# alexandreGellibert/SDR-for-Android-lib

Measured on AMD Instinct MI355X. Metric: IQ Msamples/s (16384-pt FFT+SSB) at 1/2/4/8 GPUs; % HBM roofline, higher is better.
Workload: dtype f32 (int8 CS8 in, int16 PCM out)

## Files before the change

sdr-for-android-lib_amd/csrc/ssb.hip:

```cpp
#include <hip/hip_ext.h>
#include <stdio.h>
#include <stdlib.h>

#include <vector>

#include "pulse_front.h"
#include "sdrg_internal.h"
#include "ssb_common.h"
#include "ssb_lpf_asm.h"
#include "ssb_math.h"

#pragma clang fp contract(off)

namespace sdrg {
namespace {

constexpr int WAVE = 64;

struct Chain {
    float dc;
    float a0, a1, a2, b1, b2, z1, z2;
    float target, fast, gain;
    int upper;

// ... 355 lines not shown
                st_work += __builtin_amdgcn_s_memtime() - st_a;
            }
            lds_barrier();
        }
    };
    auto run = [&](int off, auto &&body) {
        chunk_loop([&](int it) {
            const int c = it - off;
            if (c >= 0 && c < nch) body(c);
        });
    };
    if ((skip_mask >> wave) & 1) {
        chunk_loop([&](int) {});
    } else if (wave == W_DC) {
        float dc = 0.0f;
        run(1, [&](int c) {
            const float alpha = 0.9995f, one_minus = 1.0f - 0.9995f, a0 = p.lpf[0];
            if (SDRG_DC_ASM && c >= 0 && c < nch && lane < PG) {
                const f2v om2 = {one_minus, one_minus}, a02 = {a0, a0};
                const uint32_t src = lds_addr(&L.re[c & 1][my_s * ROW]), dst = lds_addr(&L.a[c % NA][my_s * ROW]);
                if (SDRG_DC_ASM == 2)
                    asm volatile(SDRG_DC_CHUNK_IL_ASM
                                 : [dc] "+v"(dc)
                                 : [src] "v"(src), [dst] "v"(dst), [alpha] "s"(alpha), [om2] "s"(om2), [a02] "s"(a02)
                                 : SDRG_CHUNK_CLOBBERS, "memory");
                else
                    asm volatile(SDRG_DC_CHUNK_ASM
                                 : [dc] "+v"(dc)
                                 : [src] "v"(src), [dst] "v"(dst), [alpha] "s"(alpha), [om2] "s"(om2), [a02] "s"(a02)
                                 : SDRG_CHUNK_CLOBBERS, "memory");
            } else if (c >= 0 && c < nch && lane < PG) {
                row_pipeline(&L.re[c & 1][my_s * ROW], &L.a[c % NA][my_s * ROW], lane < PG, [&](float (&v)[SB]) {
#pragma unroll
                    for (int q = 0; q < SB; q++) {
                        dc = alpha * dc + one_minus * v[q];
                        v[q] = a0 * (v[q] - dc);
                    }
                });
            }
        });
    } else if (wave == W_LPF) {
        float z1 = 0.0f, z2 = 0.0f;
        const bool lpf_asm_loop = LA && SDRG_LPF_ASM && S % CH == 0;
        if (s0 + my_s < n_frames) {
            z1 = state[s0 + my_s].lpf_z1;
            z2 = state[s0 + my_s].lpf_z2;
        }
        const f2v c1 = {p.lpf[1], -p.lpf[3]}, c2 = {p.lpf[2], -p.lpf[4]};
        static_assert(BUFF * 4 == SDRG_LPF_LOOP_SLOT_BYTES, "ring slot stride of the generated loop");
        if (lpf_asm_loop) {
            f2v z = {z1, z2};
            const uint32_t abase = lds_addr(&L.a[0][my_s * ROW]), ybase = lds_addr(&L.y[0][my_s * ROW]);
            const int nit = nch + 8 + LA;
            unsigned long long sv;
            int t_it, t_cc, t_r, t_yo;
            if (SDRG_LPF_INTERLEAVE)
                asm volatile(SDRG_LPF_LOOP_IL_ASM
                             : [z] "+v"(z), [sv] "=&s"(sv), [it] "=&s"(t_it), [cc] "=&s"(t_cc), [r] "=&s"(t_r), [yo] "=&s"(t_yo)
                             : [abase] "v"(abase), [ybase] "v"(ybase), [c1] "s"(c1), [c2] "s"(c2), [nit] "s"(nit), [nch] "s"(nch)
                             : SDRG_CHUNK_CLOBBERS, "v54", "memory");
            else
                asm volatile(SDRG_LPF_LOOP_ASM
                             : [z] "+v"(z), [sv] "=&s"(sv), [it] "=&s"(t_it), [cc] "=&s"(t_cc), [r] "=&s"(t_r), [yo] "=&s"(t_yo)
                             : [abase] "v"(abase), [ybase] "v"(ybase), [c1] "s"(c1), [c2] "s"(c2), [nit] "s"(nit), [nch] "s"(nch)
                             : SDRG_CHUNK_CLOBBERS, "v54", "memory");
            z1 = z.x;
            z2 = z.y;
        } else run(2 + LA, [&](int c) {
            if (c >= 0 && c < nch && lane < PG) {
                const int lim = min(CH, S - c * CH);
                if (lim == CH && SDRG_LPF_ASM) {
                    f2v z = {z1, z2};
                    const uint32_t src = lds_addr(&L.a[c % NA][my_s * ROW]), dst = lds_addr(y_row(c, my_s));
                    asm volatile(SDRG_LPF_CHUNK_ASM
                                 : [z] "+v"(z)
                                 : [src] "v"(src), [dst] "v"(dst), [c1] "s"(c1), [c2] "s"(c2)
                                 : SDRG_LPF_CHUNK_CLOBBERS, "memory");
                    z1 = z.x;
                    z2 = z.y;
                } else if (lim == CH) {
                    row_pipeline(&L.a[c % NA][my_s * ROW], y_row(c, my_s), lane < PG, [&](float (&v)[SB]) {
#pragma unroll
                        for (int q = 0; q < SB; q++) {
                            const f2v p1 = c1 * z1, p2 = c2 * z2;
                            const float y = (((v[q] + p1.x) + p2.x) + p1.y) + p2.y;
                            z2 = z1;
                            z1 = y;
                            v[q] = y;
                        }
                    });
                } else {
                    for (int q = 0; q < lim; q++) {
                        const f2v p1 = c1 * z1, p2 = c2 * z2;
                        const float y = (((L.a[c % NA][my_s * ROW + q] + p1.x) + p2.x) + p1.y) + p2.y;
                        z2 = z1;
                        z1 = y;
                        if (lane < PG) y_row(c, my_s)[q] = y;
                    }
                }
            }
        });
        if (lane < PG && s0 + my_s < n_frames) {
            state[s0 + my_s].lpf_z1 = z1;
            state[s0 + my_s].lpf_z2 = z2;
        }
    } else if (wave == W_AGC) {
        float gain = 1.0f;
        const f2v rates = {p.agc_fast, 0.00035f};
        const f2v keep = {1.0f - p.agc_fast, 1.0f - 0.00035f};
        run(4 + LA, [&](int c) {
            if (SDRG_AGC_ASM && c >= 0 && c < nch && lane < PG) {
// ... 472 lines not shown
```

sdr-for-android-lib_amd/csrc/ssb_lpf_asm.h:

```cpp
#pragma once
#define SDRG_LPF_CHUNK_ASM \
    "ds_read_b128 v[0:3], %[src] offset:0\n" \
    "ds_read_b128 v[4:7], %[src] offset:16\n" \
    "ds_read_b128 v[8:11], %[src] offset:32\n" \
    "ds_read_b128 v[12:15], %[src] offset:48\n" \
    "ds_read_b128 v[16:19], %[src] offset:64\n" \
    "ds_read_b128 v[20:23], %[src] offset:80\n" \
    "ds_read_b128 v[24:27], %[src] offset:96\n" \
    "ds_read_b128 v[28:31], %[src] offset:112\n" \
    "s_waitcnt lgkmcnt(4)\n" \
    "v_pk_mul_f32 v[48:49], %[c1], %[z] op_sel:[0,0] op_sel_hi:[1,0]\n" \
    "v_pk_mul_f32 v[50:51], %[c2], %[z] op_sel:[0,1] op_sel_hi:[1,1]\n" \
    "v_add_f32 v0, v0, v48\n" \
    "v_add_f32 v0, v0, v50\n" \
    "v_add_f32 v0, v0, v49\n" \
    "v_add_f32 v0, v0, v51\n" \
    "v_pk_mul_f32 v[48:49], %[c1], v[0:1] op_sel:[0,0] op_sel_hi:[1,0]\n" \
    "v_pk_mul_f32 v[50:51], %[c2], %[z] op_sel:[0,0] op_sel_hi:[1,0]\n" \
    "v_add_f32 v1, v1, v48\n" \
    "v_add_f32 v1, v1, v50\n" \
    "v_add_f32 v1, v1, v49\n" \
    "v_add_f32 v1, v1, v51\n" \
    "v_pk_mul_f32 v[48:49], %[c1], v[0:1] op_sel:[0,1] op_sel_hi:[1,1]\n" \
    "v_pk_mul_f32 v[50:51], %[c2], v[0:1] op_sel:[0,0] op_sel_hi:[1,0]\n" \
// ... 2934 lines not shown
    "v_pk_mov_b32 v[52:53], v[46:47], v[46:47] op_sel:[1,0]\n" \
    "s_add_u32 %[yo], %[cc], 1\n" \
    "s_cmp_ge_i32 %[yo], %[nch]\n" \
    "s_cbranch_scc1 L_drain_%=\n" \
    "ds_read_b128 v[0:3], %[abase] offset:0\n" \
    "ds_read_b128 v[4:7], %[abase] offset:16\n" \
    "ds_read_b128 v[8:11], %[abase] offset:32\n" \
    "ds_read_b128 v[12:15], %[abase] offset:48\n" \
    "ds_read_b128 v[16:19], %[abase] offset:64\n" \
    "ds_read_b128 v[20:23], %[abase] offset:80\n" \
    "ds_read_b128 v[24:27], %[abase] offset:96\n" \
    "ds_read_b128 v[28:31], %[abase] offset:112\n" \
    "s_branch L_bar8_%=\n" \
    "L_pre_%=:\n" \
    "s_cmp_lg_i32 %[cc], -1\n" \
    "s_cbranch_scc1 L_drain_%=\n" \
    "s_cmp_le_i32 %[nch], 0\n" \
    "s_cbranch_scc1 L_drain_%=\n" \
    "ds_read_b128 v[0:3], %[abase] offset:0\n" \
    "ds_read_b128 v[4:7], %[abase] offset:16\n" \
    "ds_read_b128 v[8:11], %[abase] offset:32\n" \
    "ds_read_b128 v[12:15], %[abase] offset:48\n" \
    "ds_read_b128 v[16:19], %[abase] offset:64\n" \
    "ds_read_b128 v[20:23], %[abase] offset:80\n" \
    "ds_read_b128 v[24:27], %[abase] offset:96\n" \
    "ds_read_b128 v[28:31], %[abase] offset:112\n" \
    "L_bar8_%=:\n" \
    "s_waitcnt lgkmcnt(8)\n" \
    "s_branch L_bar_%=\n" \
    "L_drain_%=:\n" \
    "s_waitcnt lgkmcnt(0)\n" \
    "L_bar_%=:\n" \
    "s_barrier\n" \
    "s_add_u32 %[it], %[it], 1\n" \
    "s_add_i32 %[cc], %[cc], 1\n" \
    "s_cmp_le_i32 %[cc], 0\n" \
    "s_cbranch_scc1 L_next_%=\n" \
    "s_add_u32 %[r], %[r], 1\n" \
    "s_cmp_eq_u32 %[r], 3\n" \
    "s_cselect_b32 %[r], 0, %[r]\n" \
    "L_next_%=:\n" \
    "s_cmp_lt_u32 %[it], %[nit]\n" \
    "s_cbranch_scc1 L_top_%=\n" \
    "s_mov_b64 exec, %[sv]\n" \
    "s_nop 4\n" \
    "v_pk_mov_b32 %[z], v[52:53], v[52:53] op_sel:[0,1]\n" \
    ""
#define SDRG_LPF_LOOP_IL_ASM \
    "s_mov_b64 %[sv], exec\n" \
    "s_mov_b64 exec, 0xffff\n" \
    "s_nop 4\n" \
    "v_pk_mov_b32 v[46:47], %[z], %[z] op_sel:[1,0]\n" \
    "v_pk_mov_b32 v[52:53], %[z], %[z] op_sel:[0,1]\n" \
    "s_mov_b32 %[it], 0\n" \
    "s_mov_b32 %[cc], -3\n" \
    "s_mov_b32 %[r], 0\n" \
    "L_top_%=:\n" \
    "s_cmp_lt_i32 %[cc], 0\n" \
    "s_cbranch_scc1 L_pre_%=\n" \
    "s_cmp_ge_i32 %[cc], %[nch]\n" \
    "s_cbranch_scc1 L_drain_%=\n" \
    "s_and_b32 %[yo], %[cc], 3\n" \
    "s_mul_i32 %[yo], %[yo], 4352\n" \
    "v_add_u32 v54, %[yo], %[ybase]\n" \
    "s_cmp_eq_u32 %[r], 0\n" \
    "s_cbranch_scc1 L_r0_%=\n" \
    "s_cmp_eq_u32 %[r], 1\n" \
    "s_cbranch_scc1 L_r1_%=\n" \
    "s_branch L_r2_%=\n" \
    "L_r0_%=:\n" \
    "s_waitcnt lgkmcnt(4)\n" \
    "v_pk_mul_f32 v[48:49], %[c1], v[46:47] op_sel:[0,1] op_sel_hi:[1,1]\n" \
    "v_pk_mul_f32 v[50:51], %[c2], v[46:47] op_sel:[0,0] op_sel_hi:[1,0]\n" \
    "v_add_f32 v0, v0, v48\n" \
    "v_add_f32 v0, v0, v50\n" \
    "v_add_f32 v0, v0, v49\n" \
    "v_add_f32 v0, v0, v51\n" \
    "v_pk_mul_f32 v[48:49], %[c1], v[0:1] op_sel:[0,0] op_sel_hi:[1,0]\n" \
    "v_pk_mul_f32 v[50:51], %[c2], v[46:47] op_sel:[0,1] op_sel_hi:[1,1]\n" \
    "v_add_f32 v1, v1, v48\n" \
    "v_add_f32 v1, v1, v50\n" \
    "v_add_f32 v1, v1, v49\n" \
    "v_add_f32 v1, v1, v51\n" \
    "v_pk_mul_f32 v[48:49], %[c1], v[0:1] op_sel:[0,1] op_sel_hi:[1,1]\n" \
    "v_pk_mul_f32 v[50:51], %[c2], v[0:1] op_sel:[0,0] op_sel_hi:[1,0]\n" \
    "v_add_f32 v2, v2, v48\n" \
    "v_add_f32 v2, v2, v50\n" \
    "v_add_f32 v2, v2, v49\n" \
    "v_add_f32 v2, v2, v51\n" \
    "v_pk_mul_f32 v[48:49], %[c1], v[2:3] op_sel:[0,0] op_sel_hi:[1,0]\n" \
    "v_pk_mul_f32 v[50:51], %[c2], v[0:1] op_sel:[0,1] op_sel_hi:[1,1]\n" \
    "v_add_f32 v3, v3, v48\n" \
    "v_add_f32 v3, v3, v50\n" \
    "v_add_f32 v3, v3, v49\n" \
    "v_add_f32 v3, v3, v51\n" \
    "ds_write_b128 v54, v[0:3] offset:0\n" \
    "ds_read_b128 v[32:35], %[abase] offset:128\n" \
    "v_pk_mul_f32 v[48:49], %[c1], v[2:3] op_sel:[0,1] op_sel_hi:[1,1]\n" \
    "v_pk_mul_f32 v[50:51], %[c2], v[2:3] op_sel:[0,0] op_sel_hi:[1,0]\n" \
    "v_add_f32 v4, v4, v48\n" \
    "v_add_f32 v4, v4, v50\n" \
    "v_add_f32 v4, v4, v49\n" \
    "v_add_f32 v4, v4, v51\n" \
    "v_pk_mul_f32 v[48:49], %[c1], v[4:5] op_sel:[0,0] op_sel_hi:[1,0]\n" \
    "v_pk_mul_f32 v[50:51], %[c2], v[2:3] op_sel:[0,1] op_sel_hi:[1,1]\n" \
    "v_add_f32 v5, v5, v48\n" \
    "v_add_f32 v5, v5, v50\n" \
    "v_add_f32 v5, v5, v49\n" \
    "v_add_f32 v5, v5, v51\n" \
    "v_pk_mul_f32 v[48:49], %[c1], v[4:5] op_sel:[0,1] op_sel_hi:[1,1]\n" \
    "v_pk_mul_f32 v[50:51], %[c2], v[4:5] op_sel:[0,0] op_sel_hi:[1,0]\n" \
    "v_add_f32 v6, v6, v48\n" \
    "v_add_f32 v6, v6, v50\n" \
    "v_add_f32 v6, v6, v49\n" \
    "v_add_f32 v6, v6, v51\n" \
    "v_pk_mul_f32 v[48:49], %[c1], v[6:7] op_sel:[0,0] op_sel_hi:[1,0]\n" \
    "v_pk_mul_f32 v[50:51], %[c2], v[4:5] op_sel:[0,1] op_sel_hi:[1,1]\n" \
    "v_add_f32 v7, v7, v48\n" \
    "v_add_f32 v7, v7, v50\n" \
    "v_add_f32 v7, v7, v49\n" \
    "v_add_f32 v7, v7, v51\n" \
    "ds_write_b128 v54, v[4:7] offset:16\n" \
    "ds_read_b128 v[36:39], %[abase] offset:144\n" \
    "v_pk_mul_f32 v[48:49], %[c1], v[6:7] op_sel:[0,1] op_sel_hi:[1,1]\n" \
    "v_pk_mul_f32 v[50:51], %[c2], v[6:7] op_sel:[0,0] op_sel_hi:[1,0]\n" \
    "v_add_f32 v8, v8, v48\n" \
    "v_add_f32 v8, v8, v50\n" \
    "v_add_f32 v8, v8, v49\n" \
    "v_add_f32 v8, v8, v51\n" \
    "v_pk_mul_f32 v[48:49], %[c1], v[8:9] op_sel:[0,0] op_sel_hi:[1,0]\n" \
    "v_pk_mul_f32 v[50:51], %[c2], v[6:7] op_sel:[0,1] op_sel_hi:[1,1]\n" \
    "v_add_f32 v9, v9, v48\n" \
    "v_add_f32 v9, v9, v50\n" \
    "v_add_f32 v9, v9, v49\n" \
    "v_add_f32 v9, v9, v51\n" \
    "v_pk_mul_f32 v[48:49], %[c1], v[8:9] op_sel:[0,1] op_sel_hi:[1,1]\n" \
    "v_pk_mul_f32 v[50:51], %[c2], v[8:9] op_sel:[0,0] op_sel_hi:[1,0]\n" \
    "v_add_f32 v10, v10, v48\n" \
    "v_add_f32 v10, v10, v50\n" \
    "v_add_f32 v10, v10, v49\n" \
    "v_add_f32 v10, v10, v51\n" \
    "v_pk_mul_f32 v[48:49], %[c1], v[10:11] op_sel:[0,0] op_sel_hi:[1,0]\n" \
    "v_pk_mul_f32 v[50:51], %[c2], v[8:9] op_sel:[0,1] op_sel_hi:[1,1]\n" \
    "v_add_f32 v11, v11, v48\n" \
    "v_add_f32 v11, v11, v50\n" \
    "v_add_f32 v11, v11, v49\n" \
    "v_add_f32 v11, v11, v51\n" \
    "ds_write_b128 v54, v[8:11] offset:32\n" \
// ... 290 lines not shown
    "v_pk_mul_f32 v[48:49], %[c1], v[6:7] op_sel:[0,1] op_sel_hi:[1,1]\n" \
    "v_pk_mul_f32 v[50:51], %[c2], v[6:7] op_sel:[0,0] op_sel_hi:[1,0]\n" \
    "v_add_f32 v8, v8, v48\n" \
    "v_add_f32 v8, v8, v50\n" \
    "v_add_f32 v8, v8, v49\n" \
    "v_add_f32 v8, v8, v51\n" \
    "v_pk_mul_f32 v[48:49], %[c1], v[8:9] op_sel:[0,0] op_sel_hi:[1,0]\n" \
    "v_pk_mul_f32 v[50:51], %[c2], v[6:7] op_sel:[0,1] op_sel_hi:[1,1]\n" \
    "v_add_f32 v9, v9, v48\n" \
    "v_add_f32 v9, v9, v50\n" \
    "v_add_f32 v9, v9, v49\n" \
    "v_add_f32 v9, v9, v51\n" \
    "v_pk_mul_f32 v[48:49], %[c1], v[8:9] op_sel:[0,1] op_sel_hi:[1,1]\n" \
    "v_pk_mul_f32 v[50:51], %[c2], v[8:9] op_sel:[0,0] op_sel_hi:[1,0]\n" \
    "v_add_f32 v10, v10, v48\n" \
    "v_add_f32 v10, v10, v50\n" \
    "v_add_f32 v10, v10, v49\n" \
    "v_add_f32 v10, v10, v51\n" \
    "v_pk_mul_f32 v[48:49], %[c1], v[10:11] op_sel:[0,0] op_sel_hi:[1,0]\n" \
    "v_pk_mul_f32 v[50:51], %[c2], v[8:9] op_sel:[0,1] op_sel_hi:[1,1]\n" \
    "v_add_f32 v11, v11, v48\n" \
    "v_add_f32 v11, v11, v50\n" \
    "v_add_f32 v11, v11, v49\n" \
    "v_add_f32 v11, v11, v51\n" \
    "ds_write_b128 v54, v[8:11] offset:224\n" \
    "ds_read_b128 v[40:43], %[abase] offset:4448\n" \
    "v_pk_mul_f32 v[48:49], %[c1], v[10:11] op_sel:[0,1] op_sel_hi:[1,1]\n" \
    "v_pk_mul_f32 v[50:51], %[c2], v[10:11] op_sel:[0,0] op_sel_hi:[1,0]\n" \
    "v_add_f32 v12, v12, v48\n" \
    "v_add_f32 v12, v12, v50\n" \
    "v_add_f32 v12, v12, v49\n" \
    "v_add_f32 v12, v12, v51\n" \
    "v_pk_mul_f32 v[48:49], %[c1], v[12:13] op_sel:[0,0] op_sel_hi:[1,0]\n" \
    "v_pk_mul_f32 v[50:51], %[c2], v[10:11] op_sel:[0,1] op_sel_hi:[1,1]\n" \
    "v_add_f32 v13, v13, v48\n" \
    "v_add_f32 v13, v13, v50\n" \
    "v_add_f32 v13, v13, v49\n" \
    "v_add_f32 v13, v13, v51\n" \
    "v_pk_mul_f32 v[48:49], %[c1], v[12:13] op_sel:[0,1] op_sel_hi:[1,1]\n" \
    "v_pk_mul_f32 v[50:51], %[c2], v[12:13] op_sel:[0,0] op_sel_hi:[1,0]\n" \
    "v_add_f32 v14, v14, v48\n" \
    "v_add_f32 v14, v14, v50\n" \
    "v_add_f32 v14, v14, v49\n" \
    "v_add_f32 v14, v14, v51\n" \
    "v_pk_mul_f32 v[48:49], %[c1], v[14:15] op_sel:[0,0] op_sel_hi:[1,0]\n" \
    "v_pk_mul_f32 v[50:51], %[c2], v[12:13] op_sel:[0,1] op_sel_hi:[1,1]\n" \
    "v_add_f32 v15, v15, v48\n" \
    "v_add_f32 v15, v15, v50\n" \
    "v_add_f32 v15, v15, v49\n" \
    "v_add_f32 v15, v15, v51\n" \
    "ds_write_b128 v54, v[12:15] offset:240\n" \
    "ds_read_b128 v[44:47], %[abase] offset:4464\n" \
    "v_pk_mov_b32 v[52:53], v[14:15], v[14:15] op_sel:[1,0]\n" \
    "s_branch L_bar1_%=\n" \
    "L_r1_%=:\n" \
    "s_waitcnt lgkmcnt(4)\n" \
    "v_pk_mul_f32 v[48:49], %[c1], v[14:15] op_sel:[0,1] op_sel_hi:[1,1]\n" \
    "v_pk_mul_f32 v[50:51], %[c2], v[14:15] op_sel:[0,0] op_sel_hi:[1,0]\n" \
    "v_add_f32 v16, v16, v48\n" \
    "v_add_f32 v16, v16, v50\n" \
    "v_add_f32 v16, v16, v49\n" \
    "v_add_f32 v16, v16, v51\n" \
    "v_pk_mul_f32 v[48:49], %[c1], v[16:17] op_sel:[0,0] op_sel_hi:[1,0]\n" \
    "v_pk_mul_f32 v[50:51], %[c2], v[14:15] op_sel:[0,1] op_sel_hi:[1,1]\n" \
    "v_add_f32 v17, v17, v48\n" \
    "v_add_f32 v17, v17, v50\n" \
    "v_add_f32 v17, v17, v49\n" \
    "v_add_f32 v17, v17, v51\n" \
    "v_pk_mul_f32 v[48:49], %[c1], v[16:17] op_sel:[0,1] op_sel_hi:[1,1]\n" \
    "v_pk_mul_f32 v[50:51], %[c2], v[16:17] op_sel:[0,0] op_sel_hi:[1,0]\n" \
    "v_add_f32 v18, v18, v48\n" \
    "v_add_f32 v18, v18, v50\n" \
    "v_add_f32 v18, v18, v49\n" \
    "v_add_f32 v18, v18, v51\n" \
    "v_pk_mul_f32 v[48:49], %[c1], v[18:19] op_sel:[0,0] op_sel_hi:[1,0]\n" \
    "v_pk_mul_f32 v[50:51], %[c2], v[16:17] op_sel:[0,1] op_sel_hi:[1,1]\n" \
    "v_add_f32 v19, v19, v48\n" \
    "v_add_f32 v19, v19, v50\n" \
    "v_add_f32 v19, v19, v49\n" \
    "v_add_f32 v19, v19, v51\n" \
    "ds_write_b128 v54, v[16:19] offset:0\n" \
    "ds_read_b128 v[0:3], %[abase] offset:4480\n" \
    "v_pk_mul_f32 v[48:49], %[c1], v[18:19] op_sel:[0,1] op_sel_hi:[1,1]\n" \
    "v_pk_mul_f32 v[50:51], %[c2], v[18:19] op_sel:[0,0] op_sel_hi:[1,0]\n" \
    "v_add_f32 v20, v20, v48\n" \
    "v_add_f32 v20, v20, v50\n" \
    "v_add_f32 v20, v20, v49\n" \
    "v_add_f32 v20, v20, v51\n" \
    "v_pk_mul_f32 v[48:49], %[c1], v[20:21] op_sel:[0,0] op_sel_hi:[1,0]\n" \
    "v_pk_mul_f32 v[50:51], %[c2], v[18:19] op_sel:[0,1] op_sel_hi:[1,1]\n" \
    "v_add_f32 v21, v21, v48\n" \
    "v_add_f32 v21, v21, v50\n" \
    "v_add_f32 v21, v21, v49\n" \
    "v_add_f32 v21, v21, v51\n" \
    "v_pk_mul_f32 v[48:49], %[c1], v[20:21] op_sel:[0,1] op_sel_hi:[1,1]\n" \
    "v_pk_mul_f32 v[50:51], %[c2], v[20:21] op_sel:[0,0] op_sel_hi:[1,0]\n" \
    "v_add_f32 v22, v22, v48\n" \
    "v_add_f32 v22, v22, v50\n" \
    "v_add_f32 v22, v22, v49\n" \
    "v_add_f32 v22, v22, v51\n" \
    "v_pk_mul_f32 v[48:49], %[c1], v[22:23] op_sel:[0,0] op_sel_hi:[1,0]\n" \
    "v_pk_mul_f32 v[50:51], %[c2], v[20:21] op_sel:[0,1] op_sel_hi:[1,1]\n" \
    "v_add_f32 v23, v23, v48\n" \
    "v_add_f32 v23, v23, v50\n" \
    "v_add_f32 v23, v23, v49\n" \
    "v_add_f32 v23, v23, v51\n" \
    "ds_write_b128 v54, v[20:23] offset:16\n" \
    "ds_read_b128 v[4:7], %[abase] offset:4496\n" \
    "v_pk_mul_f32 v[48:49], %[c1], v[22:23] op_sel:[0,1] op_sel_hi:[1,1]\n" \
    "v_pk_mul_f32 v[50:51], %[c2], v[22:23] op_sel:[0,0] op_sel_hi:[1,0]\n" \
    "v_add_f32 v24, v24, v48\n" \
    "v_add_f32 v24, v24, v50\n" \
    "v_add_f32 v24, v24, v49\n" \
    "v_add_f32 v24, v24, v51\n" \
    "v_pk_mul_f32 v[48:49], %[c1], v[24:25] op_sel:[0,0] op_sel_hi:[1,0]\n" \
    "v_pk_mul_f32 v[50:51], %[c2], v[22:23] op_sel:[0,1] op_sel_hi:[1,1]\n" \
    "v_add_f32 v25, v25, v48\n" \
    "v_add_f32 v25, v25, v50\n" \
    "v_add_f32 v25, v25, v49\n" \
    "v_add_f32 v25, v25, v51\n" \
    "v_pk_mul_f32 v[48:49], %[c1], v[24:25] op_sel:[0,1] op_sel_hi:[1,1]\n" \
    "v_pk_mul_f32 v[50:51], %[c2], v[24:25] op_sel:[0,0] op_sel_hi:[1,0]\n" \
    "v_add_f32 v26, v26, v48\n" \
    "v_add_f32 v26, v26, v50\n" \
    "v_add_f32 v26, v26, v49\n" \
    "v_add_f32 v26, v26, v51\n" \
    "v_pk_mul_f32 v[48:49], %[c1], v[26:27] op_sel:[0,0] op_sel_hi:[1,0]\n" \
    "v_pk_mul_f32 v[50:51], %[c2], v[24:25] op_sel:[0,1] op_sel_hi:[1,1]\n" \
    "v_add_f32 v27, v27, v48\n" \
    "v_add_f32 v27, v27, v50\n" \
    "v_add_f32 v27, v27, v49\n" \
    "v_add_f32 v27, v27, v51\n" \
    "ds_write_b128 v54, v[24:27] offset:32\n" \
// ... 290 lines not shown
    "v_pk_mul_f32 v[48:49], %[c1], v[22:23] op_sel:[0,1] op_sel_hi:[1,1]\n" \
    "v_pk_mul_f32 v[50:51], %[c2], v[22:23] op_sel:[0,0] op_sel_hi:[1,0]\n" \
    "v_add_f32 v24, v24, v48\n" \
    "v_add_f32 v24, v24, v50\n" \
    "v_add_f32 v24, v24, v49\n" \
    "v_add_f32 v24, v24, v51\n" \
    "v_pk_mul_f32 v[48:49], %[c1], v[24:25] op_sel:[0,0] op_sel_hi:[1,0]\n" \
    "v_pk_mul_f32 v[50:51], %[c2], v[22:23] op_sel:[0,1] op_sel_hi:[1,1]\n" \
    "v_add_f32 v25, v25, v48\n" \
    "v_add_f32 v25, v25, v50\n" \
    "v_add_f32 v25, v25, v49\n" \
    "v_add_f32 v25, v25, v51\n" \
    "v_pk_mul_f32 v[48:49], %[c1], v[24:25] op_sel:[0,1] op_sel_hi:[1,1]\n" \
    "v_pk_mul_f32 v[50:51], %[c2], v[24:25] op_sel:[0,0] op_sel_hi:[1,0]\n" \
    "v_add_f32 v26, v26, v48\n" \
    "v_add_f32 v26, v26, v50\n" \
    "v_add_f32 v26, v26, v49\n" \
    "v_add_f32 v26, v26, v51\n" \
    "v_pk_mul_f32 v[48:49], %[c1], v[26:27] op_sel:[0,0] op_sel_hi:[1,0]\n" \
    "v_pk_mul_f32 v[50:51], %[c2], v[24:25] op_sel:[0,1] op_sel_hi:[1,1]\n" \
    "v_add_f32 v27, v27, v48\n" \
    "v_add_f32 v27, v27, v50\n" \
    "v_add_f32 v27, v27, v49\n" \
    "v_add_f32 v27, v27, v51\n" \
    "ds_write_b128 v54, v[24:27] offset:224\n" \
    "ds_read_b128 v[8:11], %[abase] offset:8800\n" \
    "v_pk_mul_f32 v[48:49], %[c1], v[26:27] op_sel:[0,1] op_sel_hi:[1,1]\n" \
    "v_pk_mul_f32 v[50:51], %[c2], v[26:27] op_sel:[0,0] op_sel_hi:[1,0]\n" \
    "v_add_f32 v28, v28, v48\n" \
    "v_add_f32 v28, v28, v50\n" \
    "v_add_f32 v28, v28, v49\n" \
    "v_add_f32 v28, v28, v51\n" \
    "v_pk_mul_f32 v[48:49], %[c1], v[28:29] op_sel:[0,0] op_sel_hi:[1,0]\n" \
    "v_pk_mul_f32 v[50:51], %[c2], v[26:27] op_sel:[0,1] op_sel_hi:[1,1]\n" \
    "v_add_f32 v29, v29, v48\n" \
    "v_add_f32 v29, v29, v50\n" \
    "v_add_f32 v29, v29, v49\n" \
    "v_add_f32 v29, v29, v51\n" \
    "v_pk_mul_f32 v[48:49], %[c1], v[28:29] op_sel:[0,1] op_sel_hi:[1,1]\n" \
    "v_pk_mul_f32 v[50:51], %[c2], v[28:29] op_sel:[0,0] op_sel_hi:[1,0]\n" \
    "v_add_f32 v30, v30, v48\n" \
    "v_add_f32 v30, v30, v50\n" \
    "v_add_f32 v30, v30, v49\n" \
    "v_add_f32 v30, v30, v51\n" \
    "v_pk_mul_f32 v[48:49], %[c1], v[30:31] op_sel:[0,0] op_sel_hi:[1,0]\n" \
    "v_pk_mul_f32 v[50:51], %[c2], v[28:29] op_sel:[0,1] op_sel_hi:[1,1]\n" \
    "v_add_f32 v31, v31, v48\n" \
    "v_add_f32 v31, v31, v50\n" \
    "v_add_f32 v31, v31, v49\n" \
    "v_add_f32 v31, v31, v51\n" \
    "ds_write_b128 v54, v[28:31] offset:240\n" \
    "ds_read_b128 v[12:15], %[abase] offset:8816\n" \
    "v_pk_mov_b32 v[52:53], v[30:31], v[30:31] op_sel:[1,0]\n" \
    "s_branch L_bar1_%=\n" \
    "L_r2_%=:\n" \
    "s_waitcnt lgkmcnt(4)\n" \
    "v_pk_mul_f32 v[48:49], %[c1], v[30:31] op_sel:[0,1] op_sel_hi:[1,1]\n" \
    "v_pk_mul_f32 v[50:51], %[c2], v[30:31] op_sel:[0,0] op_sel_hi:[1,0]\n" \
    "v_add_f32 v32, v32, v48\n" \
    "v_add_f32 v32, v32, v50\n" \
    "v_add_f32 v32, v32, v49\n" \
    "v_add_f32 v32, v32, v51\n" \
    "v_pk_mul_f32 v[48:49], %[c1], v[32:33] op_sel:[0,0] op_sel_hi:[1,0]\n" \
    "v_pk_mul_f32 v[50:51], %[c2], v[30:31] op_sel:[0,1] op_sel_hi:[1,1]\n" \
    "v_add_f32 v33, v33, v48\n" \
    "v_add_f32 v33, v33, v50\n" \
    "v_add_f32 v33, v33, v49\n" \
    "v_add_f32 v33, v33, v51\n" \
    "v_pk_mul_f32 v[48:49], %[c1], v[32:33] op_sel:[0,1] op_sel_hi:[1,1]\n" \
    "v_pk_mul_f32 v[50:51], %[c2], v[32:33] op_sel:[0,0] op_sel_hi:[1,0]\n" \
    "v_add_f32 v34, v34, v48\n" \
    "v_add_f32 v34, v34, v50\n" \
    "v_add_f32 v34, v34, v49\n" \
    "v_add_f32 v34, v34, v51\n" \
    "v_pk_mul_f32 v[48:49], %[c1], v[34:35] op_sel:[0,0] op_sel_hi:[1,0]\n" \
    "v_pk_mul_f32 v[50:51], %[c2], v[32:33] op_sel:[0,1] op_sel_hi:[1,1]\n" \
    "v_add_f32 v35, v35, v48\n" \
    "v_add_f32 v35, v35, v50\n" \
    "v_add_f32 v35, v35, v49\n" \
    "v_add_f32 v35, v35, v51\n" \
    "ds_write_b128 v54, v[32:35] offset:0\n" \
    "ds_read_b128 v[16:19], %[abase] offset:8832\n" \
    "v_pk_mul_f32 v[48:49], %[c1], v[34:35] op_sel:[0,1] op_sel_hi:[1,1]\n" \
    "v_pk_mul_f32 v[50:51], %[c2], v[34:35] op_sel:[0,0] op_sel_hi:[1,0]\n" \
    "v_add_f32 v36, v36, v48\n" \
    "v_add_f32 v36, v36, v50\n" \
    "v_add_f32 v36, v36, v49\n" \
    "v_add_f32 v36, v36, v51\n" \
    "v_pk_mul_f32 v[48:49], %[c1], v[36:37] op_sel:[0,0] op_sel_hi:[1,0]\n" \
    "v_pk_mul_f32 v[50:51], %[c2], v[34:35] op_sel:[0,1] op_sel_hi:[1,1]\n" \
    "v_add_f32 v37, v37, v48\n" \
    "v_add_f32 v37, v37, v50\n" \
    "v_add_f32 v37, v37, v49\n" \
    "v_add_f32 v37, v37, v51\n" \
    "v_pk_mul_f32 v[48:49], %[c1], v[36:37] op_sel:[0,1] op_sel_hi:[1,1]\n" \
    "v_pk_mul_f32 v[50:51], %[c2], v[36:37] op_sel:[0,0] op_sel_hi:[1,0]\n" \
    "v_add_f32 v38, v38, v48\n" \
    "v_add_f32 v38, v38, v50\n" \
    "v_add_f32 v38, v38, v49\n" \
    "v_add_f32 v38, v38, v51\n" \
    "v_pk_mul_f32 v[48:49], %[c1], v[38:39] op_sel:[0,0] op_sel_hi:[1,0]\n" \
    "v_pk_mul_f32 v[50:51], %[c2], v[36:37] op_sel:[0,1] op_sel_hi:[1,1]\n" \
    "v_add_f32 v39, v39, v48\n" \
    "v_add_f32 v39, v39, v50\n" \
    "v_add_f32 v39, v39, v49\n" \
    "v_add_f32 v39, v39, v51\n" \
    "ds_write_b128 v54, v[36:39] offset:16\n" \
    "ds_read_b128 v[20:23], %[abase] offset:8848\n" \
    "v_pk_mul_f32 v[48:49], %[c1], v[38:39] op_sel:[0,1] op_sel_hi:[1,1]\n" \
    "v_pk_mul_f32 v[50:51], %[c2], v[38:39] op_sel:[0,0] op_sel_hi:[1,0]\n" \
    "v_add_f32 v40, v40, v48\n" \
    "v_add_f32 v40, v40, v50\n" \
    "v_add_f32 v40, v40, v49\n" \
    "v_add_f32 v40, v40, v51\n" \
    "v_pk_mul_f32 v[48:49], %[c1], v[40:41] op_sel:[0,0] op_sel_hi:[1,0]\n" \
    "v_pk_mul_f32 v[50:51], %[c2], v[38:39] op_sel:[0,1] op_sel_hi:[1,1]\n" \
    "v_add_f32 v41, v41, v48\n" \
    "v_add_f32 v41, v41, v50\n" \
    "v_add_f32 v41, v41, v49\n" \
    "v_add_f32 v41, v41, v51\n" \
    "v_pk_mul_f32 v[48:49], %[c1], v[40:41] op_sel:[0,1] op_sel_hi:[1,1]\n" \
    "v_pk_mul_f32 v[50:51], %[c2], v[40:41] op_sel:[0,0] op_sel_hi:[1,0]\n" \
    "v_add_f32 v42, v42, v48\n" \
    "v_add_f32 v42, v42, v50\n" \
    "v_add_f32 v42, v42, v49\n" \
    "v_add_f32 v42, v42, v51\n" \
    "v_pk_mul_f32 v[48:49], %[c1], v[42:43] op_sel:[0,0] op_sel_hi:[1,0]\n" \
    "v_pk_mul_f32 v[50:51], %[c2], v[40:41] op_sel:[0,1] op_sel_hi:[1,1]\n" \
    "v_add_f32 v43, v43, v48\n" \
    "v_add_f32 v43, v43, v50\n" \
    "v_add_f32 v43, v43, v49\n" \
    "v_add_f32 v43, v43, v51\n" \
    "ds_write_b128 v54, v[40:43] offset:32\n" \
// ... 290 lines not shown
    "v_pk_mul_f32 v[48:49], %[c1], v[38:39] op_sel:[0,1] op_sel_hi:[1,1]\n" \
    "v_pk_mul_f32 v[50:51], %[c2], v[38:39] op_sel:[0,0] op_sel_hi:[1,0]\n" \
    "v_add_f32 v40, v40, v48\n" \
    "v_add_f32 v40, v40, v50\n" \
    "v_add_f32 v40, v40, v49\n" \
    "v_add_f32 v40, v40, v51\n" \
    "v_pk_mul_f32 v[48:49], %[c1], v[40:41] op_sel:[0,0] op_sel_hi:[1,0]\n" \
    "v_pk_mul_f32 v[50:51], %[c2], v[38:39] op_sel:[0,1] op_sel_hi:[1,1]\n" \
    "v_add_f32 v41, v41, v48\n" \
    "v_add_f32 v41, v41, v50\n" \
    "v_add_f32 v41, v41, v49\n" \
    "v_add_f32 v41, v41, v51\n" \
    "v_pk_mul_f32 v[48:49], %[c1], v[40:41] op_sel:[0,1] op_sel_hi:[1,1]\n" \
    "v_pk_mul_f32 v[50:51], %[c2], v[40:41] op_sel:[0,0] op_sel_hi:[1,0]\n" \
    "v_add_f32 v42, v42, v48\n" \
    "v_add_f32 v42, v42, v50\n" \
    "v_add_f32 v42, v42, v49\n" \
    "v_add_f32 v42, v42, v51\n" \
    "v_pk_mul_f32 v[48:49], %[c1], v[42:43] op_sel:[0,0] op_sel_hi:[1,0]\n" \
    "v_pk_mul_f32 v[50:51], %[c2], v[40:41] op_sel:[0,1] op_sel_hi:[1,1]\n" \
    "v_add_f32 v43, v43, v48\n" \
    "v_add_f32 v43, v43, v50\n" \
    "v_add_f32 v43, v43, v49\n" \
    "v_add_f32 v43, v43, v51\n" \
    "ds_write_b128 v54, v[40:43] offset:224\n" \
    "ds_read_b128 v[24:27], %[abase] offset:96\n" \
    "v_pk_mul_f32 v[48:49], %[c1], v[42:43] op_sel:[0,1] op_sel_hi:[1,1]\n" \
    "v_pk_mul_f32 v[50:51], %[c2], v[42:43] op_sel:[0,0] op_sel_hi:[1,0]\n" \
    "v_add_f32 v44, v44, v48\n" \
    "v_add_f32 v44, v44, v50\n" \
    "v_add_f32 v44, v44, v49\n" \
    "v_add_f32 v44, v44, v51\n" \
    "v_pk_mul_f32 v[48:49], %[c1], v[44:45] op_sel:[0,0] op_sel_hi:[1,0]\n" \
    "v_pk_mul_f32 v[50:51], %[c2], v[42:43] op_sel:[0,1] op_sel_hi:[1,1]\n" \
    "v_add_f32 v45, v45, v48\n" \
    "v_add_f32 v45, v45, v50\n" \
    "v_add_f32 v45, v45, v49\n" \
    "v_add_f32 v45, v45, v51\n" \
    "v_pk_mul_f32 v[48:49], %[c1], v[44:45] op_sel:[0,1] op_sel_hi:[1,1]\n" \
    "v_pk_mul_f32 v[50:51], %[c2], v[44:45] op_sel:[0,0] op_sel_hi:[1,0]\n" \
    "v_add_f32 v46, v46, v48\n" \
    "v_add_f32 v46, v46, v50\n" \
    "v_add_f32 v46, v46, v49\n" \
    "v_add_f32 v46, v46, v51\n" \
    "v_pk_mul_f32 v[48:49], %[c1], v[46:47] op_sel:[0,0] op_sel_hi:[1,0]\n" \
    "v_pk_mul_f32 v[50:51], %[c2], v[44:45] op_sel:[0,1] op_sel_hi:[1,1]\n" \
    "v_add_f32 v47, v47, v48\n" \
    "v_add_f32 v47, v47, v50\n" \
    "v_add_f32 v47, v47, v49\n" \
    "v_add_f32 v47, v47, v51\n" \
    "ds_write_b128 v54, v[44:47] offset:240\n" \
    "ds_read_b128 v[28:31], %[abase] offset:112\n" \
    "v_pk_mov_b32 v[52:53], v[46:47], v[46:47] op_sel:[1,0]\n" \
    "s_branch L_bar1_%=\n" \
    "L_pre_%=:\n" \
    "s_cmp_lg_i32 %[cc], -1\n" \
    "s_cbranch_scc1 L_drain_%=\n" \
    "s_cmp_le_i32 %[nch], 0\n" \
    "s_cbranch_scc1 L_drain_%=\n" \
    "ds_read_b128 v[0:3], %[abase] offset:0\n" \
    "ds_read_b128 v[4:7], %[abase] offset:16\n" \
    "ds_read_b128 v[8:11], %[abase] offset:32\n" \
    "ds_read_b128 v[12:15], %[abase] offset:48\n" \
    "ds_read_b128 v[16:19], %[abase] offset:64\n" \
    "ds_read_b128 v[20:23], %[abase] offset:80\n" \
    "ds_read_b128 v[24:27], %[abase] offset:96\n" \
    "ds_read_b128 v[28:31], %[abase] offset:112\n" \
    "s_branch L_bar_%=\n" \
    "L_bar1_%=:\n" \
    "s_waitcnt lgkmcnt(1)\n" \
    "s_branch L_bar_%=\n" \
    "L_drain_%=:\n" \
    "s_waitcnt lgkmcnt(0)\n" \
    "L_bar_%=:\n" \
    "s_barrier\n" \
    "s_add_u32 %[it], %[it], 1\n" \
    "s_add_i32 %[cc], %[cc], 1\n" \
    "s_cmp_le_i32 %[cc], 0\n" \
    "s_cbranch_scc1 L_next_%=\n" \
    "s_add_u32 %[r], %[r], 1\n" \
    "s_cmp_eq_u32 %[r], 3\n" \
    "s_cselect_b32 %[r], 0, %[r]\n" \
    "L_next_%=:\n" \
    "s_cmp_lt_u32 %[it], %[nit]\n" \
    "s_cbranch_scc1 L_top_%=\n" \
    "s_waitcnt lgkmcnt(0)\n" \
    "s_mov_b64 exec, %[sv]\n" \
    "s_nop 4\n" \
    "v_pk_mov_b32 %[z], v[52:53], v[52:53] op_sel:[0,1]\n" \
    ""
#define SDRG_CHUNK_CLOBBERS \
    "v0", "v1", "v2", "v3", "v4", "v5", "v6", "v7", "v8", "v9", "v10", "v11", "v12", "v13", "v14", "v15", \
    "v16", "v17", "v18", "v19", "v20", "v21", "v22", "v23", "v24", "v25", "v26", "v27", "v28", "v29", "v30", "v31", \
    "v32", "v33", "v34", "v35", "v36", "v37", "v38", "v39", "v40", "v41", "v42", "v43", "v44", "v45", "v46", "v47", \
    "v48", "v49", "v50", "v51", "v52", "v53"
#define SDRG_LPF_CHUNK_CLOBBERS SDRG_CHUNK_CLOBBERS
#define SDRG_LPF_LOOP_SLOT_BYTES 4352
```

Before: 221,400.

## Restructure interleaved LPF asm loop into straight-line rotation with called barrier

Replaces the dispatch loop in the interleaved LPF inline-asm (rotation-index branches, counter updates, and separate prologue and drain paths) with a straight-line three-phase rotation. Each phase falls through to the next and reaches the shared barrier through s_call_b64/s_setpc_b64. The chunk counter and ring-slot offset updates are interleaved with the first IIR additions of each phase, so the scalar work overlaps vector math. A separate idle loop issues the remaining barriers so the count matches the other waves. This trims scalar branching and serial bookkeeping between barriers on the sequential filter wave, at the cost of subtle barrier-count and lgkmcnt correctness risk.

```diff
diff --git a/sdr-for-android-lib_amd/csrc/ssb.hip b/sdr-for-android-lib_amd/csrc/ssb.hip
--- a/sdr-for-android-lib_amd/csrc/ssb.hip
+++ b/sdr-for-android-lib_amd/csrc/ssb.hip
@@ -431,11 +431,11 @@
             f2v z = {z1, z2};
             const uint32_t abase = lds_addr(&L.a[0][my_s * ROW]), ybase = lds_addr(&L.y[0][my_s * ROW]);
             const int nit = nch + 8 + LA;
-            unsigned long long sv;
+            unsigned long long sv, t_ret;
             int t_it, t_cc, t_r, t_yo;
             if (SDRG_LPF_INTERLEAVE)
                 asm volatile(SDRG_LPF_LOOP_IL_ASM
-                             : [z] "+v"(z), [sv] "=&s"(sv), [it] "=&s"(t_it), [cc] "=&s"(t_cc), [r] "=&s"(t_r), [yo] "=&s"(t_yo)
+                             : [z] "+v"(z), [sv] "=&s"(sv), [it] "=&s"(t_it), [cc] "=&s"(t_cc), [ret] "=&s"(t_ret), [yo] "=&s"(t_yo)
                              : [abase] "v"(abase), [ybase] "v"(ybase), [c1] "s"(c1), [c2] "s"(c2), [nit] "s"(nit), [nch] "s"(nch)
                              : SDRG_CHUNK_CLOBBERS, "v54", "memory");
             else
diff --git a/sdr-for-android-lib_amd/csrc/ssb_lpf_asm.h b/sdr-for-android-lib_amd/csrc/ssb_lpf_asm.h
--- a/sdr-for-android-lib_amd/csrc/ssb_lpf_asm.h
+++ b/sdr-for-android-lib_amd/csrc/ssb_lpf_asm.h
@@ -3010,48 +3010,23 @@
     "s_nop 4\n" \
     "v_pk_mov_b32 v[46:47], %[z], %[z] op_sel:[1,0]\n" \
     "v_pk_mov_b32 v[52:53], %[z], %[z] op_sel:[0,1]\n" \
-    "s_mov_b32 %[it], 0\n" \
-    "s_mov_b32 %[cc], -3\n" \
-    "s_mov_b32 %[r], 0\n" \
-    "L_top_%=:\n" \
-    "s_cmp_lt_i32 %[cc], 0\n" \
-    "s_cbranch_scc1 L_pre_%=\n" \
-    "s_cmp_ge_i32 %[cc], %[nch]\n" \
-    "s_cbranch_scc1 L_drain_%=\n" \
-    "s_and_b32 %[yo], %[cc], 3\n" \
-    "s_mul_i32 %[yo], %[yo], 4352\n" \
-    "v_add_u32 v54, %[yo], %[ybase]\n" \
-    "s_cmp_eq_u32 %[r], 0\n" \
-    "s_cbranch_scc1 L_r0_%=\n" \
-    "s_cmp_eq_u32 %[r], 1\n" \
-    "s_cbranch_scc1 L_r1_%=\n" \
-    "s_branch L_r2_%=\n" \
+    "s_mov_b32 %[it], %[nit]\n" \
+    "s_cmp_le_i32 %[nch], 0\n" \
+    "s_cbranch_scc1 L_idle_%=\n" \
+    "s_call_b64 %[ret], L_bar_%=\n" \
+    "s_call_b64 %[ret], L_bar_%=\n" \
+    "ds_read_b128 v[0:3], %[abase] offset:0\n" \
+    "ds_read_b128 v[4:7], %[abase] offset:16\n" \
+    "ds_read_b128 v[8:11], %[abase] offset:32\n" \
+    "ds_read_b128 v[12:15], %[abase] offset:48\n" \
+    "ds_read_b128 v[16:19], %[abase] offset:64\n" \
+    "ds_read_b128 v[20:23], %[abase] offset:80\n" \
+    "ds_read_b128 v[24:27], %[abase] offset:96\n" \
+    "ds_read_b128 v[28:31], %[abase] offset:112\n" \
+    "s_mov_b32 %[cc], -1\n" \
+    "s_waitcnt lgkmcnt(4)\n" \
+    "s_branch L_ra2_%=\n" \
     "L_r0_%=:\n" \
-    "s_waitcnt lgkmcnt(4)\n" \
-    "v_pk_mul_f32 v[48:49], %[c1], v[46:47] op_sel:[0,1] op_sel_hi:[1,1]\n" \
-    "v_pk_mul_f32 v[50:51], %[c2], v[46:47] op_sel:[0,0] op_sel_hi:[1,0]\n" \
-    "v_add_f32 v0, v0, v48\n" \
-    "v_add_f32 v0, v0, v50\n" \
-    "v_add_f32 v0, v0, v49\n" \
-    "v_add_f32 v0, v0, v51\n" \
-    "v_pk_mul_f32 v[48:49], %[c1], v[0:1] op_sel:[0,0] op_sel_hi:[1,0]\n" \
-    "v_pk_mul_f32 v[50:51], %[c2], v[46:47] op_sel:[0,1] op_sel_hi:[1,1]\n" \
-    "v_add_f32 v1, v1, v48\n" \
-    "v_add_f32 v1, v1, v50\n" \
-    "v_add_f32 v1, v1, v49\n" \
-    "v_add_f32 v1, v1, v51\n" \
-    "v_pk_mul_f32 v[48:49], %[c1], v[0:1] op_sel:[0,1] op_sel_hi:[1,1]\n" \
-    "v_pk_mul_f32 v[50:51], %[c2], v[0:1] op_sel:[0,0] op_sel_hi:[1,0]\n" \
-    "v_add_f32 v2, v2, v48\n" \
-    "v_add_f32 v2, v2, v50\n" \
-    "v_add_f32 v2, v2, v49\n" \
-    "v_add_f32 v2, v2, v51\n" \
-    "v_pk_mul_f32 v[48:49], %[c1], v[2:3] op_sel:[0,0] op_sel_hi:[1,0]\n" \
-    "v_pk_mul_f32 v[50:51], %[c2], v[0:1] op_sel:[0,1] op_sel_hi:[1,1]\n" \
-    "v_add_f32 v3, v3, v48\n" \
-    "v_add_f32 v3, v3, v50\n" \
-    "v_add_f32 v3, v3, v49\n" \
-    "v_add_f32 v3, v3, v51\n" \
     "ds_write_b128 v54, v[0:3] offset:0\n" \
     "ds_read_b128 v[32:35], %[abase] offset:128\n" \
     "v_pk_mul_f32 v[48:49], %[c1], v[2:3] op_sel:[0,1] op_sel_hi:[1,1]\n" \
@@ -3448,18 +3423,22 @@
     "ds_write_b128 v54, v[12:15] offset:240\n" \
     "ds_read_b128 v[44:47], %[abase] offset:4464\n" \
     "v_pk_mov_b32 v[52:53], v[14:15], v[14:15] op_sel:[1,0]\n" \
-    "s_branch L_bar1_%=\n" \
-    "L_r1_%=:\n" \
-    "s_waitcnt lgkmcnt(4)\n" \
+    "s_waitcnt lgkmcnt(8)\n" \
+    "L_ra0_%=:\n" \
     "v_pk_mul_f32 v[48:49], %[c1], v[14:15] op_sel:[0,1] op_sel_hi:[1,1]\n" \
     "v_pk_mul_f32 v[50:51], %[c2], v[14:15] op_sel:[0,0] op_sel_hi:[1,0]\n" \
     "v_add_f32 v16, v16, v48\n" \
+    "s_add_i32 %[cc], %[cc], 1\n" \
     "v_add_f32 v16, v16, v50\n" \
+    "s_and_b32 %[yo], %[cc], 3\n" \
     "v_add_f32 v16, v16, v49\n" \
+    "s_mul_i32 %[yo], %[yo], 4352\n" \
     "v_add_f32 v16, v16, v51\n" \
+    "v_add_u32 v54, %[yo], %[ybase]\n" \
     "v_pk_mul_f32 v[48:49], %[c1], v[16:17] op_sel:[0,0] op_sel_hi:[1,0]\n" \
     "v_pk_mul_f32 v[50:51], %[c2], v[14:15] op_sel:[0,1] op_sel_hi:[1,1]\n" \
     "v_add_f32 v17, v17, v48\n" \
+    "s_cmp_ge_i32 %[cc], %[nch]\n" \
     "v_add_f32 v17, v17, v50\n" \
     "v_add_f32 v17, v17, v49\n" \
     "v_add_f32 v17, v17, v51\n" \
@@ -3475,6 +3454,10 @@
     "v_add_f32 v19, v19, v50\n" \
     "v_add_f32 v19, v19, v49\n" \
     "v_add_f32 v19, v19, v51\n" \
+    "s_cbranch_scc1 L_last_%=\n" \
+    "s_waitcnt lgkmcnt(1)\n" \
+    "s_call_b64 %[ret], L_bar_%=\n" \
+    "L_r1_%=:\n" \
     "ds_write_b128 v54, v[16:19] offset:0\n" \
     "ds_read_b128 v[0:3], %[abase] offset:4480\n" \
     "v_pk_mul_f32 v[48:49], %[c1], v[18:19] op_sel:[0,1] op_sel_hi:[1,1]\n" \
@@ -3871,18 +3854,22 @@
     "ds_write_b128 v54, v[28:31] offset:240\n" \
     "ds_read_b128 v[12:15], %[abase] offset:8816\n" \
     "v_pk_mov_b32 v[52:53], v[30:31], v[30:31] op_sel:[1,0]\n" \
-    "s_branch L_bar1_%=\n" \
-    "L_r2_%=:\n" \
-    "s_waitcnt lgkmcnt(4)\n" \
+    "s_waitcnt lgkmcnt(8)\n" \
+    "L_ra1_%=:\n" \
     "v_pk_mul_f32 v[48:49], %[c1], v[30:31] op_sel:[0,1] op_sel_hi:[1,1]\n" \
     "v_pk_mul_f32 v[50:51], %[c2], v[30:31] op_sel:[0,0] op_sel_hi:[1,0]\n" \
     "v_add_f32 v32, v32, v48\n" \
+    "s_add_i32 %[cc], %[cc], 1\n" \
     "v_add_f32 v32, v32, v50\n" \
+    "s_and_b32 %[yo], %[cc], 3\n" \
     "v_add_f32 v32, v32, v49\n" \
+    "s_mul_i32 %[yo], %[yo], 4352\n" \
     "v_add_f32 v32, v32, v51\n" \
+    "v_add_u32 v54, %[yo], %[ybase]\n" \
     "v_pk_mul_f32 v[48:49], %[c1], v[32:33] op_sel:[0,0] op_sel_hi:[1,0]\n" \
     "v_pk_mul_f32 v[50:51], %[c2], v[30:31] op_sel:[0,1] op_sel_hi:[1,1]\n" \
     "v_add_f32 v33, v33, v48\n" \
+    "s_cmp_ge_i32 %[cc], %[nch]\n" \
     "v_add_f32 v33, v33, v50\n" \
     "v_add_f32 v33, v33, v49\n" \
     "v_add_f32 v33, v33, v51\n" \
@@ -3898,6 +3885,10 @@
     "v_add_f32 v35, v35, v50\n" \
     "v_add_f32 v35, v35, v49\n" \
     "v_add_f32 v35, v35, v51\n" \
+    "s_cbranch_scc1 L_last_%=\n" \
+    "s_waitcnt lgkmcnt(1)\n" \
+    "s_call_b64 %[ret], L_bar_%=\n" \
+    "L_r2_%=:\n" \
     "ds_write_b128 v54, v[32:35] offset:0\n" \
     "ds_read_b128 v[16:19], %[abase] offset:8832\n" \
     "v_pk_mul_f32 v[48:49], %[c1], v[34:35] op_sel:[0,1] op_sel_hi:[1,1]\n" \
@@ -4294,39 +4285,55 @@
     "ds_write_b128 v54, v[44:47] offset:240\n" \
     "ds_read_b128 v[28:31], %[abase] offset:112\n" \
     "v_pk_mov_b32 v[52:53], v[46:47], v[46:47] op_sel:[1,0]\n" \
-    "s_branch L_bar1_%=\n" \
-    "L_pre_%=:\n" \
-    "s_cmp_lg_i32 %[cc], -1\n" \
-    "s_cbranch_scc1 L_drain_%=\n" \
-    "s_cmp_le_i32 %[nch], 0\n" \
-    "s_cbranch_scc1 L_drain_%=\n" \
-    "ds_read_b128 v[0:3], %[abase] offset:0\n" \
-    "ds_read_b128 v[4:7], %[abase] offset:16\n" \
-    "ds_read_b128 v[8:11], %[abase] offset:32\n" \
-    "ds_read_b128 v[12:15], %[abase] offset:48\n" \
-    "ds_read_b128 v[16:19], %[abase] offset:64\n" \
-    "ds_read_b128 v[20:23], %[abase] offset:80\n" \
-    "ds_read_b128 v[24:27], %[abase] offset:96\n" \
-    "ds_read_b128 v[28:31], %[abase] offset:112\n" \
-    "s_branch L_bar_%=\n" \
-    "L_bar1_%=:\n" \
+    "s_waitcnt lgkmcnt(8)\n" \
+    "L_ra2_%=:\n" \
+    "v_pk_mul_f32 v[48:49], %[c1], v[46:47] op_sel:[0,1] op_sel_hi:[1,1]\n" \
+    "v_pk_mul_f32 v[50:51], %[c2], v[46:47] op_sel:[0,0] op_sel_hi:[1,0]\n" \
+    "v_add_f32 v0, v0, v48\n" \
+    "s_add_i32 %[cc], %[cc], 1\n" \
+    "v_add_f32 v0, v0, v50\n" \
+    "s_and_b32 %[yo], %[cc], 3\n" \
+    "v_add_f32 v0, v0, v49\n" \
+    "s_mul_i32 %[yo], %[yo], 4352\n" \
+    "v_add_f32 v0, v0, v51\n" \
+    "v_add_u32 v54, %[yo], %[ybase]\n" \
+    "v_pk_mul_f32 v[48:49], %[c1], v[0:1] op_sel:[0,0] op_sel_hi:[1,0]\n" \
+    "v_pk_mul_f32 v[50:51], %[c2], v[46:47] op_sel:[0,1] op_sel_hi:[1,1]\n" \
+    "v_add_f32 v1, v1, v48\n" \
+    "s_cmp_ge_i32 %[cc], %[nch]\n" \
+    "v_add_f32 v1, v1, v50\n" \
+    "v_add_f32 v1, v1, v49\n" \
+    "v_add_f32 v1, v1, v51\n" \
+    "v_pk_mul_f32 v[48:49], %[c1], v[0:1] op_sel:[0,1] op_sel_hi:[1,1]\n" \
+    "v_pk_mul_f32 v[50:51], %[c2], v[0:1] op_sel:[0,0] op_sel_hi:[1,0]\n" \
+    "v_add_f32 v2, v2, v48\n" \
+    "v_add_f32 v2, v2, v50\n" \
+    "v_add_f32 v2, v2, v49\n" \
+    "v_add_f32 v2, v2, v51\n" \
+    "v_pk_mul_f32 v[48:49], %[c1], v[2:3] op_sel:[0,0] op_sel_hi:[1,0]\n" \
+    "v_pk_mul_f32 v[50:51], %[c2], v[0:1] op_sel:[0,1] op_sel_hi:[1,1]\n" \
+    "v_add_f32 v3, v3, v48\n" \
+    "v_add_f32 v3, v3, v50\n" \
+    "v_add_f32 v3, v3, v49\n" \
+    "v_add_f32 v3, v3, v51\n" \
+    "s_cbranch_scc1 L_last_%=\n" \
     "s_waitcnt lgkmcnt(1)\n" \
-    "s_branch L_bar_%=\n" \
-    "L_drain_%=:\n" \
+    "s_call_b64 %[ret], L_bar_%=\n" \
+    "s_branch L_r0_%=\n" \
+    "L_last_%=:\n" \
+    "s_sub_u32 %[it], %[nit], %[nch]\n" \
+    "s_sub_u32 %[it], %[it], 2\n" \
     "s_waitcnt lgkmcnt(0)\n" \
+    "L_idle_%=:\n" \
+    "s_cmp_le_i32 %[it], 0\n" \
+    "s_cbranch_scc1 L_end_%=\n" \
+    "s_call_b64 %[ret], L_bar_%=\n" \
+    "s_sub_u32 %[it], %[it], 1\n" \
+    "s_branch L_idle_%=\n" \
     "L_bar_%=:\n" \
     "s_barrier\n" \
-    "s_add_u32 %[it], %[it], 1\n" \
-    "s_add_i32 %[cc], %[cc], 1\n" \
-    "s_cmp_le_i32 %[cc], 0\n" \
-    "s_cbranch_scc1 L_next_%=\n" \
-    "s_add_u32 %[r], %[r], 1\n" \
-    "s_cmp_eq_u32 %[r], 3\n" \
-    "s_cselect_b32 %[r], 0, %[r]\n" \
-    "L_next_%=:\n" \
-    "s_cmp_lt_u32 %[it], %[nit]\n" \
-    "s_cbranch_scc1 L_top_%=\n" \
-    "s_waitcnt lgkmcnt(0)\n" \
+    "s_setpc_b64 %[ret]\n" \
+    "L_end_%=:\n" \
     "s_mov_b64 exec, %[sv]\n" \
     "s_nop 4\n" \
     "v_pk_mov_b32 %[z], v[52:53], v[52:53] op_sel:[0,1]\n" \
```

Result: faster. 224,300, median of 6 (+1.3%).
